# rwdavies/QUILT

Hardware: AMD Instinct MI355X
Metric: samples/sec on 2Mb region, K=50k haps, 1x coverage; dosage r2 vs CPU ref (higher is better)
Workload: dtype f64

## Files before the change

### quilt_amd/csrc/gibbs.hip

```cpp
#include "panel.hpp"

#include <chrono>
#include <functional>

#include <algorithm>
#include <cmath>
#include <cstdlib>
#include <map>
#include <memory>
#include <type_traits>

#include "gibbs_dev.hpp"
#include "gibbs_blocks.hpp"

namespace qa {
int gibbs3_waves(int Ksp, int C, int share);
void launch_gibbs3(const void *gibbs_params, hipStream_t st);
void launch_block_rate3(const void *gibbs_params, hipStream_t st);
void launch_block3(const void *gibbs_params, hipStream_t st);
void launch_resample3(const void *gibbs_params, hipStream_t st);
}

namespace {

template <int NE, int NW>
__device__ void forward_full_both(Chain<NE, NW> &ch) {
    const int G = ch.G, Ksp = ch.Ksp;
    Col<NE> a[2], e[2];
    GridStreams<Chain<NE, NW>> gs;
    for (int g = 0; g < G; g++) {
        if ((g & 63) == 0) {
            if (g) gs.store_c(ch);
            gs.load_fwd(ch, g);
        }
        const int j = g & 63;
        ch.ld(e[0], ch.eg[0] + (size_t)g * Ksp);
        ch.ld(e[1], ch.eg[1] + (size_t)g * Ksp);
        const double s0 = rl_f64(gs.t0, j), s1 = rl_f64(gs.t1, j);
#pragma unroll
        for (int h = 0; h < 2; h++) {
#pragma unroll
            for (int i = 0; i < NE; i++) {
                if (g == 0) a[h].v[i] = ch.valid[i] ? ch.prior * e[h].v[i] : 0.0;
                else a[h].v[i] = ch.valid[i] ? e[h].v[i] * (s0 * a[h].v[i] + s1 * ch.prior) : 0.0;
            }
        }
// ... 718 lines not shown
                s[3] += s_a[0].v[i] * b2.v[i];
            }
            ch.template bsum<4>(s);
            const double pA1 = mlc1 + mloc1 + log(s[0]);
            const double pA2 = mlc2 + mloc2 + log(s[1]);
            const double pB1 = mlc2 + mloc1 + log(s[2]);
            const double pB2 = mlc1 + mloc2 + log(s[3]);
            const double diff = pB1 + pB2 - pA1 - pA2;
            double probs1 = 1;
            const double probs2 = exp(diff);
            const double ps = probs1 + probs2;
            probs1 /= ps;
            const double ub = seed_shard ? stream_uniform(seed_shard, (uint64_t)p.blk_pass * (G - 1) + blk) : ru[blk];
            flip = ub > probs1;
        }
        mloc1 += log(oc1);
        mloc2 += log(oc2);
    }
    ss.store_c(ch);
    if (rr.base >= 0 && rr_dirty) rr.store(ch);
    chain_sync<NW>();
    backward_both<NE, NW, false>(ch);
}

__global__ __launch_bounds__(256) void k_happrobs(GibbsParams p) {
    const int g = blockIdx.x, c = blockIdx.y;
    const int b = threadIdx.x & 31, part = threadIdx.x >> 5;
    __shared__ double s_g[3][8][32], s_t[3][8];
    extern __shared__ __attribute__((aligned(16))) char s_dyn[];
    const int Ks = p.Ks, Ksp = p.Ksp, G = p.G;
    double *const s_gk0 = reinterpret_cast<double *>(s_dyn);
    uint32_t *const s_w = reinterpret_cast<uint32_t *>(s_gk0 + (size_t)p.nH * Ksp);
    auto gk = [&](int h, int k) -> double & { return s_gk0[(size_t)h * Ksp + k]; };
    const int32_t *which = p.which + (size_t)c * Ks;
    const size_t mat = (size_t)G * Ksp;
    for (int k = threadIdx.x; k < Ks; k += 256) {
        const int kk = which[k];
        s_w[k] = panel_word(p, g, kk, p.hm[(size_t)g * p.Kp + kk]);
        for (int h = 0; h < p.nH; h++) {
            const size_t o = ((size_t)c * p.nH + h) * mat + (size_t)g * Ksp + k;
            const double x = 1 / p.cvec[((size_t)c * 3 + h) * G + g];
            gk(h, k) = (p.alpha[o] * p.beta[o]) * x;
        }
    }
    __syncthreads();
    const int s = 32 * g, nLocal = min(32, p.T - s);
    double acc[3] = {0, 0, 0}, tot[3] = {0, 0, 0};
    if (p.nH == 2) {
        for (int k = part; k < Ks; k += 8) {
            const bool on = (s_w[k] >> b) & 1u;
            const double g0 = gk(0, k), g1 = gk(1, k);
            tot[0] += g0; tot[1] += g1;
            if (on) { acc[0] += g0; acc[1] += g1; }
        }
    } else {
        for (int k = part; k < Ks; k += 8) {
            const bool on = (s_w[k] >> b) & 1u;
            const double g0 = gk(0, k), g1 = gk(1, k), g2 = gk(2, k);
            tot[0] += g0; tot[1] += g1; tot[2] += g2;
            if (on) { acc[0] += g0; acc[1] += g1; acc[2] += g2; }
        }
    }
#pragma unroll
    for (int h = 0; h < 3; h++) {
        if (h < p.nH) {
            s_g[h][part][b] = acc[h];
            if (b == 0) s_t[h][part] = tot[h];
        }
    }
    __syncthreads();
    if (part == 0 && b < nLocal) {
// ... 22 lines not shown
}


__global__ __launch_bounds__(256) void k_happrobs_rc(GibbsParams p) {
    const int g = blockIdx.x, c = blockIdx.y;
    const int b = threadIdx.x & 31, part = threadIdx.x >> 5;
    __shared__ double s_on[3][8][32], s_all[3][8];
    __shared__ int s_cg;
    extern __shared__ __attribute__((aligned(16))) char s_dyn[];
    const int Ks = p.Ks, Ksp = p.Ksp, G = p.G;
    double *const s_gam0 = reinterpret_cast<double *>(s_dyn);
    uint32_t *const s_w0 = reinterpret_cast<uint32_t *>(s_gam0 + (size_t)p.nH * Ksp);
    int32_t *const s_which = reinterpret_cast<int32_t *>(s_w0 + 2 * (size_t)Ksp);
    auto gam = [&](int h, int k) -> double & { return s_gam0[(size_t)h * Ksp + k]; };
    auto sw = [&](int q, int k) -> uint32_t & { return s_w0[(size_t)q * Ksp + k]; };
    const int32_t *which = p.which + (size_t)c * Ks;
    const int s = 32 * g, nLocal = min(32, p.T - s);
    if (threadIdx.x < 64) {
        const int i = threadIdx.x;
        const int cs = i < nLocal ? p.rc_common[s + i] : -1;
        const unsigned long long m = __ballot(cs >= 0);
        const int first = m ? __ffsll((long long)m) - 1 : -1;
        const int cs_first = __shfl(cs, first < 0 ? 0 : first, 64);
        if (i == 0) s_cg = first < 0 ? -1 : (cs_first >> 5);
    }
    __syncthreads();
    const int cg = s_cg;
    const size_t mat = (size_t)G * Ksp;
    for (int k = threadIdx.x; k < Ks; k += 256) {
        const int kk = which[k];
        s_which[k] = kk;
        for (int q = 0; q < 2; q++) {
            const int gq = cg + q;
            sw(q, k) = (cg >= 0 && gq < p.rc_Gc) ? panel_word(p, gq, kk, p.hm[(size_t)gq * p.Kp + kk]) : 0u;
        }
        for (int h = 0; h < p.nH; h++) {
            const double *a = p.alpha + ((size_t)c * p.nH + h) * mat + (size_t)g * Ksp;
            const double *be = p.beta + ((size_t)c * p.nH + h) * mat + (size_t)g * Ksp;
            const double x = 1 / p.cvec[((size_t)c * 3 + h) * G + g];
            gam(h, k) = (a[k] * be[k]) * x;
        }
    }
    __syncthreads();
    const int snp = s + b;
    const int cs = b < nLocal ? p.rc_common[snp] : -1;
    const bool rare = b < nLocal && cs < 0;
    const bool any = rare && ((p.rc_any[(size_t)c * p.rc_words + (snp >> 5)] >> (snp & 31)) & 1u);
    const int nH = p.nH;
    double on[3] = {0, 0, 0};
    if (b < nLocal && rare && any && p.rc_pairs) {
        const int32_t *po = p.rc_pair_off + (size_t)c * (G + 1);
        const uint16_t *pp = p.rc_pairs + p.rc_pair_base[c];
        for (int i = po[g]; i < po[g + 1]; i++) {
            const uint32_t e = pp[i];
            const int k = (int)(e & 1023u);
            if ((int)(e >> 10) == b && (k & 7) == part) {
#pragma unroll
                for (int h = 0; h < 3; h++) if (h < nH) on[h] += gam(h, k);
            }
        }
    } else if (b < nLocal && (!rare || any)) {
        const int q = rare ? 0 : (cs >> 5) - cg, bit = cs & 31;
        for (int k = part; k < Ks; k += 8) {
            const bool alt = rare ? rare_has_alt(p, s_which[k], snp) : ((sw(q, k) >> bit) & 1u);
#pragma unroll
            for (int h = 0; h < 3; h++) {
                if (h < nH && alt) on[h] += gam(h, k);
// ... 96 lines not shown
    for (int k = 0; k < p.K; k++) o[k] = v[k];
}

__global__ __launch_bounds__(256) void k_pack_hap_words(const double *hap, int T, int G, int32_t *words) {
    const int g = blockIdx.x * 256 + threadIdx.x, h = blockIdx.y, c = blockIdx.z;
    if (g >= G) return;
    uint32_t w = 0;
    for (int b = 0; b < 32; b++) {
        const int t = 32 * g + b;
        if (t < T && hap[((size_t)c * T + t) * 3 + h] > 0.5) w |= 1u << b;
    }
    words[((size_t)c * 3 + h) * G + g] = (int32_t)w;
}

__global__ __launch_bounds__(256) void k_hap_major(const double *hap, int T, int nL, double *out) {
    const int t = blockIdx.x * 256 + threadIdx.x, c = blockIdx.y;
    if (t >= T) return;
    for (int h = 0; h < nL; h++) out[((size_t)c * nL + h) * T + t] = hap[((size_t)c * T + t) * 3 + h];
}

}

namespace qa {

struct GibbsScratch {
    DBuf<int32_t> which, read_off, read_ptr, base_off, u, bq, wif, block_its, first_read, H, H_class, status;
    DBuf<uint8_t> ghr, is_cat1, er_nent;
    DBuf<int32_t> dense_of;
    DBuf<size_t> eridx_off;
    ABuf<uint8_t> er_idx;
    ABuf<double> er_tab;
    DBuf<double> tabs, runif_reads, runif_shard, tm;
    ABuf<double> eMatRead, alpha, beta, eg, cvec, hap, gm, gf;
    DBuf<size_t> eread_off;
    DBuf<uint64_t> seeds;
    DBuf<uint32_t> rc_any;
    DBuf<uint16_t> rc_pairs;
    DBuf<int32_t> rc_pair_off;
    DBuf<size_t> rc_pair_base;
    DBuf<double> blk_rate2, ff_chain, per_it;
    DBuf<int32_t> blk_where, blk_tab, blk_n;
};

}

struct GibbsHolder {
    qa::GibbsScratch s;
    hipEvent_t ev[4] = {nullptr, nullptr, nullptr, nullptr};
};

namespace {

thread_local std::unique_ptr<GibbsHolder> g_gibbs;

std::vector<double> base_quality_tables() {
    std::vector<double> tabs(4 * 256);
    for (int q = 0; q < 256; q++) {
        const double en = std::pow(10, (double)(-q) / 10), ep = std::pow(10, -(double)q / 10);
        tabs[q] = 1 - en;
        tabs[256 + q] = ep / 3;
        tabs[512 + q] = en / 3;
        tabs[768 + q] = 1 - ep;
    }
    return tabs;
}

template <int NEALL, int NW>
void launch_ematread(const GibbsParams &prm, int maxR, hipStream_t st) {
    hipLaunchKernelGGL((k_ematread<NEALL, NW>), dim3((maxR + kReadsPerWave - 1) / kReadsPerWave, prm.C), dim3(64), 0, st, prm);
    QA_HIP(hipGetLastError());
}

template <int NE, int NW, bool LEAN = false, bool SEG = false>
void launch_gibbs_kernel(const GibbsParams &prm, hipStream_t st) {
    hipLaunchKernelGGL((k_gibbs<NE, NW, LEAN, SEG>), dim3(prm.C), dim3(64 * NW), 0, st, prm);
    QA_HIP(hipGetLastError());
}

template <int NE, int NW>
void launch_shard_blocks_kernel(const GibbsParams &prm, hipStream_t st) {
    hipLaunchKernelGGL((k_shard_blocks<NE, NW>), dim3(prm.C), dim3(64 * NW), 0, st, prm);
    QA_HIP(hipGetLastError());
}

int choose_gibbs_waves(int Ksp, int C, int share) {
    if (Ksp != 640) return 1;
    int nw = 1;
    if (share > 0 && (long)C * 2 <= 1024 / share) nw = 2;
    if (share == 0 && C <= 256) nw = 2;
    if (const char *forced = getenv("QA_GIBBS_NW")) {
        const int f = atoi(forced);
        if (f == 1 || f == 2 || f == 5 || f == 10) nw = f;
    }
    return nw;
}

bool use_lean_build(int C) {
// ... 17 lines not shown
        case 6: return f(int_c<6>{}, int_c<1>{});
        case 7: return f(int_c<7>{}, int_c<1>{});
        case 8: return f(int_c<8>{}, int_c<1>{});
        case 9: return f(int_c<9>{}, int_c<1>{});
        case 10: return f(int_c<10>{}, int_c<1>{});
        case 11: return f(int_c<11>{}, int_c<1>{});
        case 12: return f(int_c<12>{}, int_c<1>{});
        case 13: return f(int_c<13>{}, int_c<1>{});
        case 14: return f(int_c<14>{}, int_c<1>{});
        case 15: return f(int_c<15>{}, int_c<1>{});
        default: return f(int_c<16>{}, int_c<1>{});
    }
}

template <bool SEG>
void launch_gibbs_sweeps(const GibbsParams &prm, int nw, hipStream_t st) {
    for_chain_geometry(prm.Ksp / 64, nw, [&](auto ne, auto w) {
        constexpr int NE = decltype(ne)::value, NW = decltype(w)::value;
        if constexpr (NE == 10 && NW == 1) {
            if (use_lean_build(prm.C)) return launch_gibbs_kernel<10, 1, true, SEG>(prm, st);
        }
        launch_gibbs_kernel<NE, NW, false, SEG>(prm, st);
    });
}

void launch_shard_blocks(const GibbsParams &prm, int nw, hipStream_t st) {
    for_chain_geometry(prm.Ksp / 64, nw, [&](auto ne, auto w) { launch_shard_blocks_kernel<decltype(ne)::value, decltype(w)::value>(prm, st); });
}

void launch_gibbs(const GibbsParams &prm, int maxR, hipStream_t st, hipEvent_t *ev, bool want_probs, int nw,
                  const std::function<void()> &segmented_sweeps) {
    const int NE1 = prm.Ksp / 64;
    QA_HIP(hipEventRecord(ev[0], st));
    switch (NE1) {
        case 1: launch_ematread<1, 1>(prm, maxR, st); break;
        case 2: launch_ematread<2, 1>(prm, maxR, st); break;
        case 3: launch_ematread<3, 1>(prm, maxR, st); break;
        case 4: launch_ematread<4, 1>(prm, maxR, st); break;
        case 5: launch_ematread<5, 1>(prm, maxR, st); break;
        case 6: launch_ematread<6, 1>(prm, maxR, st); break;
        case 7: launch_ematread<7, 1>(prm, maxR, st); break;
        case 8: launch_ematread<8, 1>(prm, maxR, st); break;
        case 9: launch_ematread<9, 1>(prm, maxR, st); break;
        case 10:
            if (nw == 10) launch_ematread<10, 10>(prm, maxR, st);
            else if (nw == 5) launch_ematread<10, 5>(prm, maxR, st);
            else if (nw == 2) launch_ematread<10, 2>(prm, maxR, st);
            else launch_ematread<10, 1>(prm, maxR, st);
            break;
        case 11: launch_ematread<11, 1>(prm, maxR, st); break;
        case 12: launch_ematread<12, 1>(prm, maxR, st); break;
        case 13: launch_ematread<13, 1>(prm, maxR, st); break;
        case 14: launch_ematread<14, 1>(prm, maxR, st); break;
        case 15: launch_ematread<15, 1>(prm, maxR, st); break;
        case 16: launch_ematread<16, 1>(prm, maxR, st); break;
        default: throw std::runtime_error("Ksubset geometry not built (Ksubset / 64 rounded up must be 1..16)");
    }
    QA_HIP(hipEventRecord(ev[1], st));
    if (segmented_sweeps) segmented_sweeps();
    else launch_gibbs_sweeps<false>(prm, nw, st);
    QA_HIP(hipEventRecord(ev[2], st));
    if (want_probs) {
        const size_t lds_hp = (size_t)prm.nH * prm.Ksp * 8 + (size_t)prm.Ksp * 4;
        const size_t lds_rc = (size_t)prm.nH * prm.Ksp * 8 + (size_t)2 * prm.Ksp * 4 + (size_t)prm.Ksp * 4;
        if (prm.rc_common) hipLaunchKernelGGL(k_happrobs_rc, dim3(prm.G, prm.C), dim3(256), lds_rc, st, prm);
        else hipLaunchKernelGGL(k_happrobs, dim3(prm.G, prm.C), dim3(256), lds_hp, st, prm);
// ... 70 lines not shown
inline int32_t fold_base_quality(int32_t b, int32_t &last) {
    if (b == 0) b = last; else last = b;
    if (b > 255 || b < -255) throw std::runtime_error("|base quality| > 255");
    return b;
}

void fold_zero_base_qualities(const int32_t *rp, int R, int Jmax, int32_t *bq_eff_block) {
    int32_t last = 0;
    for (int r = 0; r < R; r++) {
        int J = rp[r + 1] - rp[r] - 1;
        if (J >= Jmax) J = Jmax;
        for (int j = 0; j <= J; j++) bq_eff_block[rp[r] + j] = fold_base_quality(bq_eff_block[rp[r] + j], last);
    }
}

std::vector<int32_t> checked_folded_qualities(int n, const int32_t *read_off, const int32_t *read_ptr, const int32_t *u, const int32_t *bq,
                                              const std::vector<int32_t> &base_off, int T, int Jmax) {
    std::vector<int32_t> bq_eff((size_t)std::max(base_off[n], 1));
    qa::parallel_for((size_t)n, qa::host_threads(), [&](size_t c) {
        const int R = read_off[c + 1] - read_off[c];
        const int32_t *rp = read_ptr + read_off[c] + c;
        const size_t b0 = (size_t)base_off[c];
        for (int i = 0; i < rp[R]; i++) {
            if (u[b0 + i] < 0 || u[b0 + i] >= T) throw std::runtime_error("read SNP index out of range");
            bq_eff[b0 + i] = bq[b0 + i];
        }
        fold_zero_base_qualities(rp, R, Jmax, bq_eff.data() + b0);
    });
    return bq_eff;
}

struct ChunkHost {
    int C, G, T, Ks, Ksp, NE, nH, n_its, nw, er_nt, er_padb, rc_words, totR, totB, maxR = 0;
    bool want_probs, want_pairs;
    bool aliased = false;
    size_t etot = 0, ixtot = 0;
    std::vector<int32_t> base_off, which0, bq_eff, dense_of, n_dense;
    std::vector<size_t> eoff, ixoff;
    std::vector<uint8_t> ghr;
    std::vector<uint32_t> rc_any;
    std::vector<int32_t> rep;
    std::vector<int64_t> hbase;
};

ChunkHost chunk_layout(qa_panel_t *pn, const qa_rare_common *rc, const qa_gibbs_opts_t *o, const GibbsLaunch &L) {
    ChunkHost h;
    const int C = h.C = L.C;
    h.G = rc ? rc->G_all : pn->G; h.T = rc ? rc->T_all : pn->T; h.Ks = o->Ks;
    h.Ksp = (h.Ks + 63) / 64 * 64; h.NE = h.Ksp / 64;
    h.nH = o->ff != 0.0 ? 3 : 2;
    h.rc_words = rc ? (h.T + 31) / 32 : 0;
    h.n_its = o->n_gibbs_burn_in_its + o->n_gibbs_sample_its;
    h.totR = L.a.read_off[C];
    h.want_probs = wants_probs(L.a, o);
    h.want_pairs = rc && h.want_probs && h.Ks <= 1024;
    h.nw = o->ff != 0.0 ? qa::gibbs3_waves(h.Ksp, C, pn->sharers()) : choose_gibbs_waves(h.Ksp, C, pn->exclusive ? 0 : pn->share);
    h.er_nt = 64 * h.nw; h.er_padb = padb_of(h.NE / h.nw);
    h.rc_any.assign((size_t)C * h.rc_words, 0u);
    h.base_off.assign(C + 1, 0); h.which0.resize((size_t)C * h.Ks);
    h.eoff.resize(C); h.ixoff.resize(C);
    h.ghr.assign((size_t)C * h.G, 0);
    h.dense_of.assign(std::max(h.totR, 1), -1);
    h.n_dense.assign(C, 0);
    for (int c = 0; c < C; c++) {
        const int R = L.a.read_off[c + 1] - L.a.read_off[c];
        h.maxR = std::max(h.maxR, R);
        const int32_t *rp = L.a.read_ptr + L.a.read_off[c] + c;
        h.base_off[c + 1] = h.base_off[c] + rp[R];
        h.ixoff[c] = h.ixtot;
        h.ixtot += (size_t)R * h.er_nt * h.er_padb;
    }
    h.totB = h.base_off[C];
    h.bq_eff.resize((size_t)std::max(h.totB, 1));
    return h;
}

void find_shared_reads(const GibbsLaunch &L, ChunkHost &h) {
    const int32_t *read_off = L.a.read_off, *read_ptr = L.a.read_ptr;
    const auto &base_off = h.base_off;
    h.rep.resize(h.C); h.hbase.resize(h.C);
    std::map<int32_t, int32_t> first_of;
// ... 146 lines not shown
    std::vector<std::vector<uint32_t>> keys((size_t)C);
    qa::parallel_for((size_t)C, qa::host_threads(), [&](size_t c) {
        auto &kv = keys[c];
        for (int k = 0; k < Ks; k++) {
            const int v = h.which0[c * Ks + k];
            for (int64_t i = rc->h_rare_ptr[v]; i < rc->h_rare_ptr[v + 1]; i++) kv.push_back(((uint32_t)rc->h_rare_snp[i] << 10) | (uint32_t)k);
        }
        std::sort(kv.begin(), kv.end());
    });
    for (int c = 0; c < C; c++) pbase[(size_t)c + 1] = pbase[(size_t)c] + keys[(size_t)c].size();
    std::vector<uint16_t> pairs(std::max<size_t>(pbase[(size_t)C], 1));
    std::vector<int32_t> poff((size_t)C * (G + 1), 0);
    for (int c = 0; c < C; c++) {
        const auto &kv = keys[(size_t)c];
        int32_t *po = poff.data() + (size_t)c * (G + 1);
        size_t i = 0;
        for (int g = 0; g < G; g++) {
            po[g] = (int32_t)i;
            while (i < kv.size() && (int)((kv[i] >> 10) >> 5) == g) {
                pairs[pbase[(size_t)c] + i] = (uint16_t)((((kv[i] >> 10) & 31u) << 10) | (kv[i] & 1023u));
                i++;
            }
        }
        po[G] = (int32_t)i;
    }
    S.rc_pairs.ensure(pairs.size()); S.rc_pairs.upload(pairs.data(), pairs.size(), st);
    S.rc_pair_off.ensure(poff.size()); S.rc_pair_off.upload(poff.data(), poff.size(), st);
    S.rc_pair_base.ensure((size_t)C); S.rc_pair_base.upload(pbase.data(), (size_t)C, st);
}

void carve_arena(qa::GibbsScratch &S, qa::Arena &arena, size_t arena_need, const ChunkHost &h) {
    const size_t mat = (size_t)h.C * h.nH * h.G * h.Ksp;
    S.er_idx.arena = S.er_tab.arena = &arena;
    S.eMatRead.arena = S.alpha.arena = S.beta.arena = S.eg.arena = S.cvec.arena = S.hap.arena = S.gm.arena = S.gf.arena = &arena;
    arena.require(arena_need);
    arena.reset();
    S.eMatRead.ensure(std::max<size_t>(h.etot, 1));
    S.er_idx.ensure(std::max<size_t>(h.ixtot, 1));
    S.er_tab.ensure(std::max<size_t>((size_t)h.totR * 64, 1));
    S.alpha.ensure(mat); S.beta.ensure(mat); S.eg.ensure(mat);
    S.cvec.ensure((size_t)h.C * 3 * h.G);
    if (h.want_probs) {
        S.hap.ensure((size_t)h.C * h.T * 3); S.gm.ensure((size_t)h.C * h.T * 3); S.gf.ensure((size_t)h.C * h.T * 3);
    }
}

GibbsParams fill_params(const qa::GibbsScratch &S, const qa_panel_t *pn, const qa_rare_common *rc, const qa_gibbs_opts_t *o,
                        const GibbsLaunch &L, const ChunkHost &h, hipStream_t st) {
    const int C = h.C;
    GibbsParams prm{};
    prm.hm = pn->hm.p; prm.B = pn->B.p; prm.sp_off = pn->sp_off.p; prm.sp_k = pn->sp_k.p;
    prm.sp_word = pn->sp_word.p; prm.sigma = S.tm.p; prm.Kp = pn->Kp; prm.G = h.G; prm.T = h.T;
    prm.nMaxDH = pn->nMaxDH; prm.ref_error = pn->ref_error;
    prm.C = C; prm.Ks = h.Ks; prm.Ksp = h.Ksp; prm.NE = h.NE; prm.which = S.which.p;
    prm.read_off = S.read_off.p; prm.read_ptr = S.read_ptr.p; prm.base_off = S.base_off.p;
    prm.u = S.u.p; prm.bq = S.bq.p; prm.wif = S.wif.p; prm.grid_has_read = S.ghr.p;
    prm.pR_tab = S.tabs.p; prm.pA_tab = S.tabs.p + 512;
    prm.Jmax = o->Jmax; prm.inv_maxdiff = 1 / o->maxDifferenceBetweenReads; prm.rescale = o->rescale_eMatRead_t;
    prm.n_its = h.n_its; prm.n_burn_in = o->n_gibbs_burn_in_its; prm.block_its = S.block_its.p;
    prm.n_block = o->perform_block_gibbs ? o->n_block_gibbs_iterations : 0;
    prm.do_shard = o->do_shard_block_gibbs; prm.init_iteratively = o->gibbs_initialize_iteratively;
    prm.disable_read_category_usage = o->disable_read_category_usage;
    prm.class_sum_cutoff = o->class_sum_cutoff;
    prm.nH = h.nH;
    prm.it_begin = 0; prm.it_end = h.n_its;
    prm.ff = o->ff;
    if (o->per_it_out) {
        QA_HIP(hipMemsetAsync(S.per_it.p, 0, sizeof(double) * C * h.n_its * 8, st));
        prm.per_it = S.per_it.p;
    }
    if (L.ff_chain) prm.ff_chain = S.ff_chain.p;
    prm.runif_reads = S.runif_reads.p; prm.first_read = S.first_read.p; prm.runif_shard = S.runif_shard.p;
    prm.seed_reads = L.a.seed_reads ? S.seeds.p : nullptr;
    prm.seed_shard = (L.a.seed_reads && L.a.seed_shard) ? S.seeds.p + C : nullptr;
    prm.eMatRead = S.eMatRead.p; prm.eread_off = S.eread_off.p; prm.is_cat1 = S.is_cat1.p; prm.er_nent = S.er_nent.p;
    prm.er_idx = S.er_idx.p; prm.eridx_off = S.eridx_off.p; prm.er_tab = S.er_tab.p; prm.dense_of = S.dense_of.p;
    prm.er_nt = h.er_nt; prm.er_padb = h.er_padb;
    prm.alpha = S.alpha.p; prm.beta = S.beta.p; prm.eg = S.eg.p; prm.cvec = S.cvec.p;
    prm.H = S.H.p; prm.H_class = S.H_class.p; prm.status = S.status.p;
    prm.hapProbs = S.hap.p; prm.genProbsM = S.gm.p; prm.genProbsF = S.gf.p;
    if (rc) {
        prm.rc_common = rc->common_index.p; prm.rc_rare_ptr = rc->rare_ptr.p; prm.rc_rare_snp = rc->rare_snp.p;
        prm.rc_any = S.rc_any.p; prm.rc_words = h.rc_words; prm.rc_Gc = pn->G;
        if (h.want_pairs) { prm.rc_pairs = S.rc_pairs.p; prm.rc_pair_off = S.rc_pair_off.p; prm.rc_pair_base = S.rc_pair_base.p; }
    }
    return prm;
}

std::vector<int> block_pass_sweeps(const qa_gibbs_opts_t *o, int n_its) {
    std::vector<int> passes;
    if (o->perform_block_gibbs)
        for (int i = 0; i < o->n_block_gibbs_iterations; i++) {
            const int b = o->block_gibbs_iterations[i];
            if (b >= 0 && b < n_its && std::find(passes.begin(), passes.end(), b) == passes.end()) passes.push_back(b);
        }
    std::sort(passes.begin(), passes.end());
    return passes;
}

void block_tables(const qa_gibbs_opts_t *o, const GibbsLaunch &L, const ChunkHost &h, const std::vector<double> &rate2,
                  const std::vector<int32_t> &seg_status, int n_thr, std::vector<int32_t> &h_where, std::vector<int32_t> &h_tab,
                  std::vector<int32_t> &h_n) {
    const int C = h.C, G = h.G;
    const int32_t *read_off = L.a.read_off;
    h_where.assign((size_t)C * G, -1); h_tab.assign((size_t)C * 4 * G, 0); h_n.assign(C, 0);
    qa::parallel_for((size_t)C, n_thr, [&](size_t c) {
        const int R = read_off[c + 1] - read_off[c];
        if (seg_status[c] != 0) return;
        if (R < 1 || (h.nH == 2 && G < 3)) {
            if (h.nH == 2) { h_n[c] = 1; h_tab[c * 4 * G + G] = G - 1; h_where[c * G + G - 1] = 0; }
            return;
        }
        const std::vector<int32_t> blocked = qa::define_blocked_grids(
// ... 352 lines not shown
                    const int32_t *rp = read_ptr + read_off[c] + c;
                    size_t n_long = 0;
                    if (!rc) {
                        for (size_t r = 0; r < R; r++) n_long += std::min(rp[r + 1] - rp[r], o->Jmax + 1) > kMaxPatternBits;
                    } else {
                        std::fill(any.begin(), any.end(), 0u);
                        for (int k = 0; k < Ks; k++) {
                            const int v = a.which[(size_t)c * Ks + k] - 1;
                            if (v < 0 || v >= pn->K) throw std::runtime_error("which_haps_to_use out of range");
                            for (int64_t i = rc->h_rare_ptr[v]; i < rc->h_rare_ptr[v + 1]; i++) {
                                const int t = rc->h_rare_snp[i];
                                any[t >> 5] |= 1u << (t & 31);
                            }
                        }
                        const int32_t *cu = a.u + base_of[o->reads_same_as ? o->reads_same_as[c] : c];
                        for (size_t r = 0; r < R; r++) {
                            const int nb_r = std::min(rp[r + 1] - rp[r], o->Jmax + 1);
                            int n_inf = 0;
                            for (int j = 0; j < nb_r; j++) {
                                const int t = cu[rp[r] + j];
                                if (t < 0 || t >= T) throw std::runtime_error("read SNP index out of range");
                                n_inf += rc->h_common_index[t] >= 0 || ((any[t >> 5] >> (t & 31)) & 1u);
                            }
                            n_long += n_inf > kMaxPatternBits;
                        }
                    }
                    n_long_of[c] = n_long;
                }
            });
        }
        for (int c = 0; c < n_chain; c++) {
            const size_t R = read_off[c + 1] - read_off[c];
            adds[c] = R * (pat_bytes + 512) + n_long_of[c] * Ksp * 8 + (size_t)(o->ff != 0.0 ? 9 : 6) * G * Ksp * 8 + (size_t)3 * G * 8 +
                      (want_probs ? (size_t)9 * T * 8 : 0) + 8192;
        }
        int n_launch = 1;
        {
            size_t need = (size_t)1 << 20;
            for (int c = 0, first = 1; c < n_chain; c++, first = 0) {
                if (!first && need + adds[c] > budget) { n_launch++; need = (size_t)1 << 20; }
                need += adds[c];
            }
        }
        const int target = (n_chain + n_launch - 1) / n_launch;
        int c0 = 0, ret = QA_OK;
        while (c0 < n_chain) {
            size_t need = (size_t)1 << 20;
            int c1 = c0;
            while (c1 < n_chain && c1 - c0 < target) {
                if (c1 > c0 && need + adds[c1] > budget) break;
                need += adds[c1];
                c1++;
            }
            const int st = gibbs_chunk(pn, need, rc, o, launch_slice(a, o, base_of, G, T, c0, c1));
            if (st < 0) return st;
            if (st == QA_UNDERFLOW) ret = QA_UNDERFLOW;
            c0 = c1;
        }
        return ret;
    });
}

}

extern "C" {

int qa_gibbs_batch(qa_panel_t *pn, const qa_gibbs_opts_t *o, int32_t n_chain, const int32_t *which_haps_to_use_1based,
                   const int32_t *read_off, const int32_t *read_ptr, const int32_t *u, const int32_t *bq,
                   const int32_t *wif, const double *runif_reads, const int32_t *first_read,
                   const double *runif_shard, int32_t *H, int32_t *H_class, double *hapProbs_t,
                   double *genProbsM_t, double *genProbsF_t, int32_t *underflow_problem, double *state_out,
                   const uint64_t *seed_reads, const uint64_t *seed_shard) {
    const GibbsCall a{which_haps_to_use_1based, read_off, read_ptr, u, bq, wif, runif_reads, first_read, runif_shard, H, H_class,
                      hapProbs_t, genProbsM_t, genProbsF_t, underflow_problem, state_out, seed_reads, seed_shard};
    return gibbs_batch_impl(pn, nullptr, o, n_chain, a);
}

int qa_gibbs_batch_rare_common(qa_panel_t *pn, const qa_rare_common_t *rc, const qa_gibbs_opts_t *o, int32_t n_chain,
                               const int32_t *which_haps_to_use_1based, const int32_t *read_off, const int32_t *read_ptr,
                               const int32_t *u, const int32_t *bq, const int32_t *wif, const double *runif_reads,
                               const int32_t *first_read, const double *runif_shard, int32_t *H, int32_t *H_class,
                               double *hapProbs_t, double *genProbsM_t, double *genProbsF_t,
                               int32_t *underflow_problem, double *state_out, const uint64_t *seed_reads,
                               const uint64_t *seed_shard) {
    if (!rc || !pn) {
        qa::set_error("qa_gibbs_batch_rare_common: null argument");
        return QA_ERR_INVALID;
    }
    if (rc->K != pn->K || rc->device != pn->device) {
        qa::set_error("qa_gibbs_batch_rare_common: the rare/common handle belongs to another panel or device");
        return QA_ERR_INVALID;
    }
    const GibbsCall a{which_haps_to_use_1based, read_off, read_ptr, u, bq, wif, runif_reads, first_read, runif_shard, H, H_class,
                      hapProbs_t, genProbsM_t, genProbsF_t, underflow_problem, state_out, seed_reads, seed_shard};
    return gibbs_batch_impl(pn, rc, o, n_chain, a);
}

int qa_rare_common_create(qa_panel_t *pn, int32_t nSNPs_all, const uint8_t *snp_is_common, const int64_t *rare_ptr,
                          const int32_t *rare_snp_1based, const double *transMatRate_t_all, qa_rare_common_t **out) {
    if (!qa::device_ready()) return QA_ERR_NO_DEVICE;
    if (!pn || !snp_is_common || !rare_ptr || !transMatRate_t_all || !out || nSNPs_all < pn->T) {
        qa::set_error("qa_rare_common_create: null argument or fewer SNPs than the panel has");
        return QA_ERR_INVALID;
    }
    return qa::guarded([&] {
        QA_HIP(hipSetDevice(pn->device));
        std::unique_ptr<qa_rare_common> rc(new qa_rare_common());
        rc->device = pn->device; rc->K = pn->K; rc->T_all = nSNPs_all; rc->G_all = (nSNPs_all + 31) / 32;
        rc->h_common_index.assign(nSNPs_all, -1);
        int n_common = 0;
        for (int t = 0; t < nSNPs_all; t++) if (snp_is_common[t]) rc->h_common_index[t] = n_common++;
        if (n_common != pn->T) throw std::runtime_error("sum(snp_is_common) differs from the panel's number of SNPs");
        const int64_t n_rare = rare_ptr[pn->K];
        if (rare_ptr[0] != 0 || n_rare < 0 || (n_rare > 0 && !rare_snp_1based)) throw std::runtime_error("bad rare_per_hap_info CSR");
        rc->h_rare_ptr.assign(rare_ptr, rare_ptr + pn->K + 1);
        rc->h_rare_snp.resize(n_rare);
        for (int k = 0; k < pn->K; k++) {
            if (rare_ptr[k + 1] < rare_ptr[k]) throw std::runtime_error("bad rare_per_hap_info CSR");
            if (rare_ptr[k + 1] > n_rare) throw std::runtime_error("rare_per_hap_info CSR: a row ends beyond the last entry");
            for (int64_t i = rare_ptr[k]; i < rare_ptr[k + 1]; i++) {
                const int t = rare_snp_1based[i] - 1;
                if (t < 0 || t >= nSNPs_all || snp_is_common[t]) throw std::runtime_error("rare_per_hap_info names a SNP that is not rare");
                if (i > rare_ptr[k] && t <= rc->h_rare_snp[i - 1]) throw std::runtime_error("rare_per_hap_info must ascend within a haplotype");
                rc->h_rare_snp[i] = t;
            }
        }
        const int G = rc->G_all;
        rc->h_sigma.resize(std::max(G - 1, 0)); rc->h_tm1.resize(std::max(G - 1, 0));
// ... 180 lines not shown
```

### quilt_amd/csrc/gibbs_dev.hpp

```cpp
#pragma once

#include "panel.hpp"

#include <cstdint>

namespace {

struct GibbsParams {
    const uint8_t *hm;
    const int32_t *B;
    const int32_t *sp_off;
    const int32_t *sp_k;
    const uint32_t *sp_word;
    const double *sigma;
    int Kp, G, T, nMaxDH;
    double ref_error;
    int C;
    int Ks, Ksp, NE;
    const int32_t *which;
    const int32_t *read_off;
    const int32_t *read_ptr;
    const int32_t *base_off;
    const int32_t *u;
    const int32_t *bq;
// ... 20 lines not shown
    uint8_t *er_idx;
    const size_t *eridx_off;
    double *er_tab;
    const int32_t *dense_of;
    int er_nt, er_padb;
    uint8_t *is_cat1;
    uint8_t *er_nent;
    double *alpha, *beta, *eg;
    double *cvec;
    int32_t *H;
    int32_t *H_class;
    int32_t *status;
    double *hapProbs, *genProbsM, *genProbsF;
    const int32_t *rc_common;
    const int64_t *rc_rare_ptr;
    const int32_t *rc_rare_snp;
    const uint32_t *rc_any;
    int rc_words, rc_Gc;
    const int32_t *rc_pair_off;
    const size_t *rc_pair_base;
    const uint16_t *rc_pairs;
    int it_begin, it_end;
    int rebuild;
    int lean3;
    const int32_t *blk_where;
    const int32_t *blk_tab;
    const int32_t *blk_n;
    double *blk_rate2;
    int blk_pass, blk_n_pass;
    int defer_resample;
    double ff;
    const double *ff_chain;
    double *per_it;
};

__device__ __forceinline__ bool rare_has_alt(const GibbsParams &p, int hap, int snp) {
    int64_t lo = p.rc_rare_ptr[hap], hi = p.rc_rare_ptr[hap + 1];
    while (lo < hi) {
        const int64_t mid = (lo + hi) >> 1;
        const int v = p.rc_rare_snp[mid];
        if (v == snp) return true;
        if (v < snp) lo = mid + 1; else hi = mid;
    }
    return false;
}

template <int CTRL, int ROW_MASK>
__device__ __forceinline__ double dpp_get(double v) {
    int lo = __double2loint(v), hi = __double2hiint(v);
    lo = __builtin_amdgcn_update_dpp(0, lo, CTRL, ROW_MASK, 0xf, true);
    hi = __builtin_amdgcn_update_dpp(0, hi, CTRL, ROW_MASK, 0xf, true);
    return __hiloint2double(hi, lo);
}
__device__ __forceinline__ double wsum(double v) {
    v += dpp_get<0x111, 0xf>(v);
    v += dpp_get<0x112, 0xf>(v);
    v += dpp_get<0x114, 0xf>(v);
    v += dpp_get<0x118, 0xf>(v);
    v += dpp_get<0x142, 0xa>(v);
    v += dpp_get<0x143, 0xc>(v);
    const int lo = __builtin_amdgcn_readlane(__double2loint(v), 63);
    const int hi = __builtin_amdgcn_readlane(__double2hiint(v), 63);
    return __hiloint2double(hi, lo);
}
__device__ __forceinline__ void wsum2(double &a, double &b) {
    const auto lo = __builtin_amdgcn_permlane32_swap(__double2loint(a), __double2loint(b), false, false);
// ... 34 lines not shown
    a = lane_of(v, 15); b = lane_of(v, 47); c = lane_of(v, 31); d = lane_of(v, 63);
}
__device__ __forceinline__ double wmax(double v) {
#pragma unroll
    for (int o = 32; o > 0; o >>= 1) v = fmax(v, __shfl_xor(v, o, 64));
    return v;
}

__device__ __forceinline__ double stream_uniform(uint64_t seed, uint64_t i) {
    uint64_t z = seed + (i + 1) * 0x9E3779B97F4A7C15ull;
    z = (z ^ (z >> 30)) * 0xBF58476D1CE4E5B9ull;
    z = (z ^ (z >> 27)) * 0x94D049BB133111EBull;
    z = z ^ (z >> 31);
    return (double)(z >> 11) * (1.0 / 9007199254740992.0);
}

__device__ __forceinline__ uint32_t panel_word(const GibbsParams &p, int g, int k, int code) {
    if (code > 0) return (uint32_t)p.B[(size_t)g * p.nMaxDH + (code - 1)];
    int lo = p.sp_off[g], hi = p.sp_off[g + 1] - 1;
    while (lo < hi) {
        int mid = (lo + hi) >> 1;
        if (p.sp_k[mid] < k) lo = mid + 1; else hi = mid;
    }
    return p.sp_word[lo];
}

__device__ __forceinline__ double rl_f64(double v, int j) {
    const int lo = __builtin_amdgcn_readlane(__double2loint(v), j);
    const int hi = __builtin_amdgcn_readlane(__double2hiint(v), j);
    return __hiloint2double(hi, lo);
}
__device__ __forceinline__ int rl_i32(int v, int j) { return __builtin_amdgcn_readlane(v, j); }

constexpr int kReadsPerWave = 32;
constexpr int kMaxPatternBits = 5;
constexpr int padb_of(int ne) { return ne <= 4 ? 4 : ne <= 8 ? 8 : ne <= 12 ? 12 : 16; }

template <int NEALL, int NW>
__global__ __launch_bounds__(64) void k_ematread(GibbsParams p) {
    constexpr int NE = NEALL / NW, PADB = padb_of(NE), NT = 64 * NW;
    const int c = blockIdx.y, lane = threadIdx.x;
    const int R = p.read_off[c + 1] - p.read_off[c];
    const int r0 = blockIdx.x * kReadsPerWave;
    if (r0 >= R) return;
    const int32_t *rp = p.read_ptr + p.read_off[c] + c;
    const int32_t *u = p.u + p.base_off[c], *bq = p.bq + p.base_off[c];
    const int32_t *which = p.which + (size_t)c * p.Ks;
    int kk[NEALL];
#pragma unroll
    for (int i = 0; i < NEALL; i++) {
        const int k = lane + 64 * i;
        kk[i] = (k < p.Ks) ? which[k] : -1;
    }
    int g_prev = -1;
    uint32_t w[NEALL];
    const double e1 = 1 - p.ref_error, e0 = p.ref_error;
    const int nblk = min(kReadsPerWave, R - r0);
    static_assert(kReadsPerWave < 64, "lane l holds the offset of read r0 + l, lane nblk the block's end");
    const int my_s = (lane <= nblk) ? rp[r0 + lane] : 0;
    const int my_dense = (lane < nblk) ? p.dense_of[p.read_off[c] + r0 + lane] : -1;
    const int b_end = rl_i32(my_s, nblk);
    int chunk0 = rl_i32(my_s, 0), c_u = 0, c_b = 0;
    double c_R = 0, c_A = 0;
    auto load_chunk = [&](int base) {
        chunk0 = base;
        const int idx = base + lane;
        const bool ok = idx < b_end;
        c_u = ok ? u[idx] : 0;
        c_b = ok ? bq[idx] : 0;
        const int ab = c_b < 0 ? -c_b : c_b;
        c_R = p.pR_tab[(c_b > 0 ? 256 : 0) + ab];
        c_A = p.pA_tab[(c_b > 0 ? 256 : 0) + ab];
    };
    load_chunk(chunk0);
    for (int r = r0; r < r0 + nblk; r++) {
        double v[NEALL];
        uint32_t pat[NEALL];
#pragma unroll
        for (int i = 0; i < NEALL; i++) { v[i] = 1.0; pat[i] = 0; }
        const int s = rl_i32(my_s, r - r0);
// ... 10 lines not shown
            if (p.rc_common) {
                const int all_snp = snp;
                snp = p.rc_common[all_snp];
                if (snp < 0) {
                    if (b == 0) continue;
                    const double pR = rl_f64(c_R, li), pA = rl_f64(c_A, li);
                    const double xe1 = e0 * pA + e1 * pR;
                    const bool any = (p.rc_any[(size_t)c * p.rc_words + (all_snp >> 5)] >> (all_snp & 31)) & 1u;
                    if (!any) {
                        if (!p.rescale) {
#pragma unroll
                            for (int i = 0; i < NEALL; i++) v[i] *= xe1;
                            tv *= xe1;
                        }
                        continue;
                    }
                    const double ratio = (e1 * pA + e0 * pR) / xe1;
#pragma unroll
                    for (int i = 0; i < NEALL; i++) {
                        const uint32_t bit = (kk[i] >= 0 && rare_has_alt(p, kk[i], all_snp)) ? 1u : 0u;
                        v[i] *= xe1;
                        if (bit) v[i] *= ratio;
                        pat[i] |= bit << min(n_inf, 7);
                    }
                    tv *= xe1;
                    if ((lane >> min(n_inf, 31)) & 1) tv *= ratio;
                    n_inf++;
                    continue;
                }
            }
            const int g = snp >> 5;
            if (g != g_prev) {
#pragma unroll
                for (int i = 0; i < NEALL; i++) {
                    w[i] = 0;
                    if (kk[i] >= 0) w[i] = panel_word(p, g, kk[i], p.hm[(size_t)g * p.Kp + kk[i]]);
                }
                g_prev = g;
            }
            if (b == 0) continue;
            const double pR = rl_f64(c_R, li), pA = rl_f64(c_A, li);
            const double f1 = (e1 * pA + (1 - e1) * pR), f0 = (e0 * pA + (1 - e0) * pR);
#pragma unroll
            for (int i = 0; i < NEALL; i++) {
                const uint32_t bit = (w[i] >> (snp & 31)) & 1u;
                v[i] *= bit ? f1 : f0;
                pat[i] |= bit << min(n_inf, 7);
            }
            tv *= ((lane >> min(n_inf, 31)) & 1) ? f1 : f0;
            n_inf++;
        }
        bool degenerate = false;
        double d1 = 1.0;
        if (p.rescale) {
            double x = 0;
#pragma unroll
            for (int i = 0; i < NEALL; i++) if (kk[i] >= 0 && v[i] > x) x = v[i];
            x = wmax(x);
            d1 = 1 / x;
            degenerate = isinf(x) || x == 0 || isinf(d1);
            if (degenerate) {
#pragma unroll
                for (int i = 0; i < NEALL; i++) v[i] = 1;
                tv = 1;
            } else {
#pragma unroll
                for (int i = 0; i < NEALL; i++) {
                    v[i] *= d1;
                    if (v[i] < p.inv_maxdiff) v[i] = p.inv_maxdiff;
                }
// ... 325 lines not shown
```

### quilt_amd/csrc/panel.hip

```cpp
#include <chrono>
#include "panel.hpp"

#include <mutex>

#include <algorithm>
#include <cmath>
#include <memory>

namespace qa {

static thread_local char g_err[1024] = "";

void set_error(const char *fmt, ...) {
    va_list ap;
    va_start(ap, fmt);
    vsnprintf(g_err, sizeof g_err, fmt, ap);
    va_end(ap);
}

static int usable_devices() {
    int n = 0;
    if (hipGetDeviceCount(&n) != hipSuccess) return 0;
    int ok = 0;
    for (int i = 0; i < n; i++) {
// ... 66 lines not shown
}

void profile_add(int kernel, double ms, double alg_bytes, double start_ms, double units, double serial, double workgroups) {
    if (kernel < 0 || kernel >= PK_COUNT) return;
    std::lock_guard<std::mutex> lock(g_profile_mutex);
    g_profile[kernel].ms += ms;
    g_profile[kernel].bytes += alg_bytes;
    g_profile[kernel].units += units;
    g_profile[kernel].serial += serial;
    g_profile[kernel].workgroups += workgroups;
    g_profile[kernel].launches += 1;
    if (start_ms >= 0) g_profile[kernel].busy.emplace_back(start_ms, start_ms + ms);
}

static const char *const kProfileNames[PK_COUNT] = {
    "k_emat", "k_fwd", "k_bwd", "k_dosage", "k_ematread", "k_gibbs", "k_happrobs", "k_fwd64", "k_bwd64", "k_topk",
    "k_fwd<double>", "k_bwd<double>", "k_gibbs3", "k_block3", "k_select", "k_best_run", "k_fwd64d", "k_bwd64d",
    "k_gibbs<10, 1, true>"};

__global__ void k_special_chunk_index(const int32_t *sp_off, const int32_t *sp_k, const int32_t *sp_grids, int n_chunks,
                                      int32_t *chunk_at) {
    const int i = blockIdx.y, c = blockIdx.x * blockDim.x + threadIdx.x;
    if (c >= n_chunks) return;
    const int g = sp_grids[i];
    int lo = sp_off[g], hi = sp_off[g + 1];
    const int k0 = c * 16;
    while (lo < hi) {
        const int mid = (lo + hi) >> 1;
        if (sp_k[mid] < k0) lo = mid + 1; else hi = mid;
    }
    chunk_at[(size_t)i * n_chunks + c] = lo + 16 * i;
}

void finish_panel_tables(qa_panel *p) {
    const int G = p->G;
    std::vector<int32_t> gidx(G, -1), grids;
    for (int g = 0; g < G; g++)
        if (p->h_sp_off[g + 1] > p->h_sp_off[g]) { gidx[g] = (int32_t)grids.size(); grids.push_back(g); }
    p->n_sp_grids = (int)grids.size();
    p->sp_gidx.alloc(G);
    p->sp_gidx.upload(gidx.data(), G, p->stream);
    const int n_chunks = (p->K + 8191) / 8192 * 512;
    p->sp_chunk_at.alloc(std::max<size_t>((size_t)p->n_sp_grids * n_chunks, 1));
    if (p->n_sp_grids > 0) {
        DBuf<int32_t> d_grids(grids.size());
        d_grids.upload(grids.data(), grids.size(), p->stream);
        hipLaunchKernelGGL(k_special_chunk_index, dim3((n_chunks + 255) / 256, p->n_sp_grids), dim3(256), 0, p->stream,
                           p->sp_off.p, p->sp_k.p, d_grids.p, n_chunks, p->sp_chunk_at.p);
        QA_HIP(hipGetLastError());
        QA_HIP(hipStreamSynchronize(p->stream));
    }
    p->tm1.alloc(std::max(G - 1, 1));
    p->tm1.upload(p->h_tm1.data(), std::max(G - 1, 0), p->stream);
    QA_HIP(hipStreamSynchronize(p->stream));
}

}

extern "C" {

int qa_profile_count(void) { return qa::PK_COUNT; }

const char *qa_profile_name(int32_t kernel) {
    return (kernel >= 0 && kernel < qa::PK_COUNT) ? qa::kProfileNames[kernel] : "";
}

int qa_profile_get_workgroups(int32_t kernel, double *workgroups) {
    if (kernel < 0 || kernel >= qa::PK_COUNT) return QA_ERR_INVALID;
// ... 432 lines not shown
```

### quilt_amd/csrc/panel.hpp

```cpp
#pragma once

#include "common.hpp"

struct qa_panel {
    int K = 0, G = 0, T = 0, nMaxDH = 0, nrow = 0;
    int Kp = 0;
    double ref_error = 0;
    int device = 0;
    qa::DBuf<uint8_t> hm;
    qa::DBuf<int32_t> B;
    qa::DBuf<int32_t> sp_off;
    qa::DBuf<int32_t> sp_k;
    qa::DBuf<uint32_t> sp_word;
    qa::DBuf<double> sigma;
    qa::DBuf<double> tm1;
    qa::DBuf<int32_t> sp_gidx, sp_chunk_at;
    int n_sp_grids = 0;
    qa::DBuf<double> IE;
    bool ie_derived = true;
    int share = 1;
    bool rank_fp64 = true;
    bool dosage_fp64 = false;
    bool sum_order_ref = false;
    bool sum_order_batched = false;
    bool sum_order_grid0_ltr = false;
    int n_special = 0;
    std::vector<double> h_sigma, h_tm1;
    std::vector<int32_t> h_sp_off;
    hipStream_t stream = nullptr;
    hipStream_t pass_stream = nullptr;
    hipStream_t gibbs_stream = nullptr;
    qa::Arena arena;
    bool exclusive = false;
    qa::DeviceGate *gate() { return exclusive ? &qa::device_gate(device) : nullptr; }
    qa::Arena &A() { return exclusive ? qa::device_gate(device).arena : arena; }
    void require_scratch(size_t bytes) {
        if (!exclusive) { arena.require(bytes); return; }
        qa::DeviceGate &g = qa::device_gate(device);
        std::lock_guard<std::mutex> lk(g.mu);
        g.grow_arena(bytes);
    }
    size_t plan_budget() {
        if (!exclusive) return arena.budget_shared(share);
        qa::DeviceGate &g = qa::device_gate(device);
        std::lock_guard<std::mutex> lk(g.mu);
        return g.arena.budget_shared(1);
    }
    int sharers() const { return exclusive ? 1 : share; }
    qa::Arena aux;
    struct Scratch;
    Scratch *scratch = nullptr;
    ~qa_panel();
};

namespace qa {
void finish_panel_tables(qa_panel *p);
void drop_pass_scratch(qa_panel *p);
__attribute__((visibility("hidden"))) int gamma_column_check(const qa_panel *p, const char *who);
}

struct qa_rare_common {
    int device = 0, K = 0, T_all = 0, G_all = 0;
    qa::DBuf<int32_t> common_index;
    qa::DBuf<int64_t> rare_ptr;
    qa::DBuf<int32_t> rare_snp;
    std::vector<int64_t> h_rare_ptr;
    std::vector<int32_t> h_rare_snp;
    std::vector<int32_t> h_common_index;
    std::vector<double> h_sigma, h_tm1;
};
```

Baseline: 36.86.

## Precompute per-chain subset panel words once per call via transposed code table

Adds a transposed haplotype code table (hmT) built once per panel, plus a kernel that decodes the panel word for every (chain, grid, selected hap) into a per-chain scratch buffer at the start of each Gibbs batch. The ematread, happrobs and rare/common kernels then read these precomputed words instead of calling panel_word on the gathered hm bytes each time. This removes repeated scattered byte gathers and repeated decoding work, at the cost of extra arena memory (C*G*Ksp*4 bytes), an extra kernel launch, and a panel-level transpose. It also adds a test hook entry point that exposes the word computation.

```diff
diff --git a/quilt_amd/csrc/gibbs.hip b/quilt_amd/csrc/gibbs.hip
--- a/quilt_amd/csrc/gibbs.hip
+++ b/quilt_amd/csrc/gibbs.hip
@@ -12,6 +12,7 @@
 
 #include "gibbs_dev.hpp"
 #include "gibbs_blocks.hpp"
+#include "gibbs_testhook.h"
 
 namespace qa {
 int gibbs3_waves(int Ksp, int C, int share);
@@ -796,11 +797,10 @@
     double *const s_gk0 = reinterpret_cast<double *>(s_dyn);
     uint32_t *const s_w = reinterpret_cast<uint32_t *>(s_gk0 + (size_t)p.nH * Ksp);
     auto gk = [&](int h, int k) -> double & { return s_gk0[(size_t)h * Ksp + k]; };
-    const int32_t *which = p.which + (size_t)c * Ks;
+    const uint32_t *sw_g = p.sw + ((size_t)c * p.sw_G + g) * Ksp;
     const size_t mat = (size_t)G * Ksp;
     for (int k = threadIdx.x; k < Ks; k += 256) {
-        const int kk = which[k];
-        s_w[k] = panel_word(p, g, kk, p.hm[(size_t)g * p.Kp + kk]);
+        s_w[k] = sw_g[k];
         for (int h = 0; h < p.nH; h++) {
             const size_t o = ((size_t)c * p.nH + h) * mat + (size_t)g * Ksp + k;
             const double x = 1 / p.cvec[((size_t)c * 3 + h) * G + g];
@@ -889,7 +889,7 @@
         s_which[k] = kk;
         for (int q = 0; q < 2; q++) {
             const int gq = cg + q;
-            sw(q, k) = (cg >= 0 && gq < p.rc_Gc) ? panel_word(p, gq, kk, p.hm[(size_t)gq * p.Kp + kk]) : 0u;
+            sw(q, k) = (cg >= 0 && gq < p.rc_Gc) ? p.sw[((size_t)c * p.sw_G + gq) * Ksp + k] : 0u;
         }
         for (int h = 0; h < p.nH; h++) {
             const double *a = p.alpha + ((size_t)c * p.nH + h) * mat + (size_t)g * Ksp;
@@ -1052,6 +1052,7 @@
     ABuf<double> er_tab;
     DBuf<double> tabs, runif_reads, runif_shard, tm;
     ABuf<double> eMatRead, alpha, beta, eg, cvec, hap, gm, gf;
+    ABuf<uint32_t> sw;
     DBuf<size_t> eread_off;
     DBuf<uint64_t> seeds;
     DBuf<uint32_t> rc_any;
@@ -1083,6 +1084,11 @@
         tabs[768 + q] = 1 - ep;
     }
     return tabs;
+}
+
+void launch_small_words(const GibbsParams &prm, hipStream_t st) {
+    hipLaunchKernelGGL(k_small_words, dim3((prm.sw_G + kWordTile - 1) / kWordTile, prm.C), dim3(256), 0, st, prm);
+    QA_HIP(hipGetLastError());
 }
 
 template <int NEALL, int NW>
@@ -1166,6 +1172,7 @@
                   const std::function<void()> &segmented_sweeps) {
     const int NE1 = prm.Ksp / 64;
     QA_HIP(hipEventRecord(ev[0], st));
+    launch_small_words(prm, st);
     switch (NE1) {
         case 1: launch_ematread<1, 1>(prm, maxR, st); break;
         case 2: launch_ematread<2, 1>(prm, maxR, st); break;
@@ -1302,6 +1309,7 @@
 
 struct ChunkHost {
     int C, G, T, Ks, Ksp, NE, nH, n_its, nw, er_nt, er_padb, rc_words, totR, totB, maxR = 0;
+    int Gpanel;
     bool want_probs, want_pairs;
     bool aliased = false;
     size_t etot = 0, ixtot = 0;
@@ -1317,6 +1325,7 @@
     ChunkHost h;
     const int C = h.C = L.C;
     h.G = rc ? rc->G_all : pn->G; h.T = rc ? rc->T_all : pn->T; h.Ks = o->Ks;
+    h.Gpanel = pn->G;
     h.Ksp = (h.Ks + 63) / 64 * 64; h.NE = h.Ksp / 64;
     h.nH = o->ff != 0.0 ? 3 : 2;
     h.rc_words = rc ? (h.T + 31) / 32 : 0;
@@ -1529,6 +1538,7 @@
 void carve_arena(qa::GibbsScratch &S, qa::Arena &arena, size_t arena_need, const ChunkHost &h) {
     const size_t mat = (size_t)h.C * h.nH * h.G * h.Ksp;
     S.er_idx.arena = S.er_tab.arena = &arena;
+    S.sw.arena = &arena;
     S.eMatRead.arena = S.alpha.arena = S.beta.arena = S.eg.arena = S.cvec.arena = S.hap.arena = S.gm.arena = S.gf.arena = &arena;
     arena.require(arena_need);
     arena.reset();
@@ -1537,6 +1547,7 @@
     S.er_tab.ensure(std::max<size_t>((size_t)h.totR * 64, 1));
     S.alpha.ensure(mat); S.beta.ensure(mat); S.eg.ensure(mat);
     S.cvec.ensure((size_t)h.C * 3 * h.G);
+    S.sw.ensure((size_t)h.C * h.Gpanel * h.Ksp);
     if (h.want_probs) {
         S.hap.ensure((size_t)h.C * h.T * 3); S.gm.ensure((size_t)h.C * h.T * 3); S.gf.ensure((size_t)h.C * h.T * 3);
     }
@@ -1576,6 +1587,7 @@
     prm.alpha = S.alpha.p; prm.beta = S.beta.p; prm.eg = S.eg.p; prm.cvec = S.cvec.p;
     prm.H = S.H.p; prm.H_class = S.H_class.p; prm.status = S.status.p;
     prm.hapProbs = S.hap.p; prm.genProbsM = S.gm.p; prm.genProbsF = S.gf.p;
+    prm.sw = S.sw.p; prm.sw_G = pn->G; prm.hmT = pn->hmT.p; prm.Gp = pn->Gp;
     if (rc) {
         prm.rc_common = rc->common_index.p; prm.rc_rare_ptr = rc->rare_ptr.p; prm.rc_rare_snp = rc->rare_snp.p;
         prm.rc_any = S.rc_any.p; prm.rc_words = h.rc_words; prm.rc_Gc = pn->G;
@@ -1994,7 +2006,7 @@
         for (int c = 0; c < n_chain; c++) {
             const size_t R = read_off[c + 1] - read_off[c];
             adds[c] = R * (pat_bytes + 512) + n_long_of[c] * Ksp * 8 + (size_t)(o->ff != 0.0 ? 9 : 6) * G * Ksp * 8 + (size_t)3 * G * 8 +
-                      (want_probs ? (size_t)9 * T * 8 : 0) + 8192;
+                      (size_t)pn->G * Ksp * 4 + (want_probs ? (size_t)9 * T * 8 : 0) + 8192;
         }
         int n_launch = 1;
         {
@@ -2056,6 +2068,34 @@
     const GibbsCall a{which_haps_to_use_1based, read_off, read_ptr, u, bq, wif, runif_reads, first_read, runif_shard, H, H_class,
                       hapProbs_t, genProbsM_t, genProbsF_t, underflow_problem, state_out, seed_reads, seed_shard};
     return gibbs_batch_impl(pn, rc, o, n_chain, a);
+}
+
+int qa_gibbs_small_panel_words(qa_panel_t *pn, int32_t n_chain, int32_t Ks, const int32_t *which_haps_to_use_1based, uint32_t *words) {
+    if (!qa::device_ready()) return QA_ERR_NO_DEVICE;
+    if (!pn || !which_haps_to_use_1based || !words || n_chain <= 0 || Ks <= 0 || Ks > QA_KSUBSET_MAX) {
+        qa::set_error("qa_gibbs_small_panel_words: null argument, no chain, or Ksubset outside 1..%d", QA_KSUBSET_MAX);
+        return QA_ERR_INVALID;
+    }
+    return qa::guarded([&] {
+        QA_HIP(hipSetDevice(pn->device));
+        const int Ksp = (Ks + 63) / 64 * 64;
+        std::vector<int32_t> which0((size_t)n_chain * Ks);
+        for (size_t i = 0; i < which0.size(); i++) {
+            which0[i] = which_haps_to_use_1based[i] - 1;
+            if (which0[i] < 0 || which0[i] >= pn->K) throw std::runtime_error("which_haps_to_use out of range");
+        }
+        const size_t n = (size_t)n_chain * pn->G * Ksp;
+        qa::DBuf<int32_t> d_which(which0.size());
+        qa::DBuf<uint32_t> d_sw(n);
+        d_which.upload(which0.data(), which0.size(), pn->stream);
+        GibbsParams prm{};
+        prm.B = pn->B.p; prm.sp_off = pn->sp_off.p; prm.sp_k = pn->sp_k.p; prm.sp_word = pn->sp_word.p;
+        prm.nMaxDH = pn->nMaxDH; prm.C = n_chain; prm.Ks = Ks; prm.Ksp = Ksp; prm.which = d_which.p;
+        prm.sw = d_sw.p; prm.sw_G = pn->G; prm.hmT = pn->hmT.p; prm.Gp = pn->Gp;
+        launch_small_words(prm, pn->stream);
+        d_sw.download(words, n, pn->stream);
+        return QA_OK;
+    });
 }
 
 int qa_rare_common_create(qa_panel_t *pn, int32_t nSNPs_all, const uint8_t *snp_is_common, const int64_t *rare_ptr,
diff --git a/quilt_amd/csrc/gibbs_dev.hpp b/quilt_amd/csrc/gibbs_dev.hpp
--- a/quilt_amd/csrc/gibbs_dev.hpp
+++ b/quilt_amd/csrc/gibbs_dev.hpp
@@ -76,6 +76,9 @@
     double ff;
     const double *ff_chain;
     double *per_it;
+    uint32_t *sw;
+    const uint8_t *hmT;
+    int sw_G, Gp;
 };
 
 __device__ __forceinline__ bool rare_has_alt(const GibbsParams &p, int hap, int snp) {
@@ -176,6 +179,34 @@
 }
 __device__ __forceinline__ int rl_i32(int v, int j) { return __builtin_amdgcn_readlane(v, j); }
 
+constexpr int kWordTile = qa::kCodeTile;
+static_assert(kWordTile % 16 == 0, "a row's codes of a tile are whole 16-byte pieces");
+__global__ __launch_bounds__(256) void k_small_words(GibbsParams p) {
+    constexpr int PITCH = kWordTile + 4;
+    __shared__ __attribute__((aligned(16))) uint8_t s_code[256 * PITCH];
+    const int c = blockIdx.y, g0 = blockIdx.x * kWordTile, t = threadIdx.x;
+    const int32_t *which = p.which + (size_t)c * p.Ks;
+    uint32_t *out = p.sw + (size_t)c * p.sw_G * p.Ksp;
+    const int ng = min(kWordTile, p.sw_G - g0);
+    for (int k0 = 0; k0 < p.Ksp; k0 += 256) {
+        if (k0) __syncthreads();
+        for (int i = t; i < 256 * (kWordTile / 16); i += 256) {
+            const int row = i / (kWordTile / 16), q = i % (kWordTile / 16), k = k0 + row;
+            uint4 v = make_uint4(0, 0, 0, 0);
+            if (k < p.Ks) v = *reinterpret_cast<const uint4 *>(p.hmT + (size_t)which[k] * p.Gp + g0 + 16 * q);
+            uint32_t *d = reinterpret_cast<uint32_t *>(s_code + row * PITCH + 16 * q);
+            d[0] = v.x; d[1] = v.y; d[2] = v.z; d[3] = v.w;
+        }
+        __syncthreads();
+        const int k = k0 + t;
+        if (k >= p.Ksp) continue;
+        const int kk = (k < p.Ks) ? which[k] : -1;
+#pragma unroll 8
+        for (int j = 0; j < ng; j++)
+            out[(size_t)(g0 + j) * p.Ksp + k] = (kk >= 0) ? panel_word(p, g0 + j, kk, s_code[t * PITCH + j]) : 0u;
+    }
+}
+
 constexpr int kReadsPerWave = 32;
 constexpr int kMaxPatternBits = 5;
 constexpr int padb_of(int ne) { return ne <= 4 ? 4 : ne <= 8 ? 8 : ne <= 12 ? 12 : 16; }
@@ -190,6 +221,7 @@
     const int32_t *rp = p.read_ptr + p.read_off[c] + c;
     const int32_t *u = p.u + p.base_off[c], *bq = p.bq + p.base_off[c];
     const int32_t *which = p.which + (size_t)c * p.Ks;
+    const uint32_t *sw = p.sw + (size_t)c * p.sw_G * p.Ksp + lane;
     int kk[NEALL];
 #pragma unroll
     for (int i = 0; i < NEALL; i++) {
@@ -266,10 +298,7 @@
             const int g = snp >> 5;
             if (g != g_prev) {
 #pragma unroll
-                for (int i = 0; i < NEALL; i++) {
-                    w[i] = 0;
-                    if (kk[i] >= 0) w[i] = panel_word(p, g, kk[i], p.hm[(size_t)g * p.Kp + kk[i]]);
-                }
+                for (int i = 0; i < NEALL; i++) w[i] = sw[(size_t)g * p.Ksp + 64 * i];
                 g_prev = g;
             }
             if (b == 0) continue;
diff --git a/quilt_amd/csrc/gibbs_testhook.h b/quilt_amd/csrc/gibbs_testhook.h
--- /dev/null
+++ b/quilt_amd/csrc/gibbs_testhook.h
@@ -0,0 +1,15 @@
+#ifndef QA_GIBBS_TESTHOOK_H
+#define QA_GIBBS_TESTHOOK_H
+#include <stdint.h>
+#include "../../include/quilt_amd.h"
+#ifdef __cplusplus
+extern "C" {
+#endif
+
+int qa_gibbs_small_panel_words(qa_panel_t *panel, int32_t n_chain, int32_t Ks, const int32_t *which_haps_to_use_1based,
+                               uint32_t *words);
+
+#ifdef __cplusplus
+}
+#endif
+#endif
diff --git a/quilt_amd/csrc/panel.hip b/quilt_amd/csrc/panel.hip
--- a/quilt_amd/csrc/panel.hip
+++ b/quilt_amd/csrc/panel.hip
@@ -122,8 +122,27 @@
     chunk_at[(size_t)i * n_chunks + c] = lo + 16 * i;
 }
 
+__global__ __launch_bounds__(256) void k_transpose_codes(const uint8_t *hm, int K, int Kp, int G, int Gp, uint8_t *hmT) {
+    __shared__ uint8_t s[kCodeTile][kCodeTile + 4];
+    const int g0 = blockIdx.x * kCodeTile, k0 = blockIdx.y * kCodeTile;
+    for (int i = threadIdx.x; i < kCodeTile * kCodeTile; i += 256) {
+        const int g = g0 + i / kCodeTile, kc = i % kCodeTile;
+        s[kc][i / kCodeTile] = g < G ? hm[(size_t)g * Kp + k0 + kc] : (uint8_t)0;
+    }
+    __syncthreads();
+    for (int i = threadIdx.x; i < kCodeTile * kCodeTile; i += 256) {
+        const int k = k0 + i / kCodeTile, gc = i % kCodeTile;
+        if (k < K) hmT[(size_t)k * Gp + g0 + gc] = s[i / kCodeTile][gc];
+    }
+}
+
 void finish_panel_tables(qa_panel *p) {
     const int G = p->G;
+    p->Gp = (G + kCodeTile - 1) / kCodeTile * kCodeTile;
+    p->hmT.alloc((size_t)p->K * p->Gp);
+    hipLaunchKernelGGL(k_transpose_codes, dim3(p->Gp / kCodeTile, (p->K + kCodeTile - 1) / kCodeTile), dim3(256), 0, p->stream,
+                       p->hm.p, p->K, p->Kp, G, p->Gp, p->hmT.p);
+    QA_HIP(hipGetLastError());
     std::vector<int32_t> gidx(G, -1), grids;
     for (int g = 0; g < G; g++)
         if (p->h_sp_off[g + 1] > p->h_sp_off[g]) { gidx[g] = (int32_t)grids.size(); grids.push_back(g); }
diff --git a/quilt_amd/csrc/panel.hpp b/quilt_amd/csrc/panel.hpp
--- a/quilt_amd/csrc/panel.hpp
+++ b/quilt_amd/csrc/panel.hpp
@@ -8,6 +8,8 @@
     double ref_error = 0;
     int device = 0;
     qa::DBuf<uint8_t> hm;
+    int Gp = 0;
+    qa::DBuf<uint8_t> hmT;
     qa::DBuf<int32_t> B;
     qa::DBuf<int32_t> sp_off;
     qa::DBuf<int32_t> sp_k;
@@ -54,6 +56,7 @@
 };
 
 namespace qa {
+constexpr int kCodeTile = 64;
 void finish_panel_tables(qa_panel *p);
 void drop_pass_scratch(qa_panel *p);
 __attribute__((visibility("hidden"))) int gamma_column_check(const qa_panel *p, const char *who);
```

After: 37.14 (median of 6 runs). About the same (+0.8%).
